# oleg-savchenko/jax_nbody_emulator_with_dj

Measured on AMD Instinct MI355X. Metric: voxels/sec (disp+vel) on 512^3 box, ndiv=4, higher is better.
Workload: dtype f32-equivalent: f16x3 split MFMA (3 f16 MFMAs per product, f32 accumulate)

## Files before the change

jax_nbody_emulator_with_dj_amd/csrc/nbe_kernels_head.h:

```cpp
constexpr int HNZ_ZRUN = 32;
constexpr int HNZ_MAXCH = 4;
constexpr int HNZ_R = 4;
constexpr int HNZ_TAPU = 4 * HNZ_R;
constexpr int HNZ_WG = 9 * HNZ_TAPU;
constexpr int HNZ_WC = 3 * HNZ_WG;
constexpr int HNZ_WS = 2 * HNZ_TAPU;
constexpr int HNZ_SBASE = HNZ_MAXCH * HNZ_WC;
constexpr int HNZ_XBASE = HNZ_SBASE + HNZ_MAXCH * HNZ_WS;
constexpr int HNZ_LDS_UNITS = HNZ_XBASE + 2 * HQ_XB;
constexpr int HNZ_SP = HP_ROWS * HP_COLS;
static_assert(8 * HNZ_SP <= HQ_XB, "the skip's patch fits a patch buffer");

__global__ __launch_bounds__(512, 1) void conv_h3nz_kernel(ConvKArgs a) {
    constexpr int R = HNZ_R, TAPU = HNZ_TAPU, WG = HNZ_WG, WC = HNZ_WC, XBASE = HNZ_XBASE, NT = 2, NW = 8;
    f32x4* lds = lds_h3;
    const half8* L8 = (const half8*)lds_h3;
    const int tid = threadIdx.x;
    const int lane = tid & 63;
    const int wave = __builtin_amdgcn_readfirstlane(tid >> 6);
    const int c = lane & 15, q = lane >> 4, kh = q & 1, ks = q >> 1;

    const int nrun = (a.Dv + a.zrun - 1) / a.zrun;
    const int tile = xcd_tile(blockIdx.x, a.ntiles);
    const int zr = tile % nrun, tyx = tile / nrun;
    const int ty = tyx / a.tnx, tx = tyx - ty * a.tnx;
    const int y0 = ty * HP_ROWS, x0 = tx * HP_COLS, z0 = zr * a.zrun;
    const int zn = min(a.zrun, a.Dv - z0);
    const int nchunk = a.nchunk, nskip = a.nskip;
    const long plane = (long)a.H * a.W * 16;
    const long to = (((long)z0 * a.H + y0) * a.W + x0) * 16;

    unsigned xoff[3];
    bool xval[3];
#pragma unroll
    for (int t = 0; t < 3; ++t) {
        const int k = (wave + NW * t) % 6;
        const int u = k * 64 + lane;
        xval[t] = u < HP_PL;
        const int uu = xval[t] ? u : HP_PL - 1;
        const int row = uu / HP_RS, col = uu - row * HP_RS;
        xoff[t] = (unsigned)(row * a.W + col) * 16u;
    }
    const unsigned soff = (unsigned)((2 * (wave & 3) + (lane >> 5) + 1) * a.W + (lane & 31) + 1) * 16u;
    auto fetch = [&](int p, int k, int buf) {
        const ConvGroupSrc e = a.gs[k];
        const char* xs = e.x + to + (long)p * plane;
        const char* dxs = e.dx + to + (long)p * plane;
        f32x4* xb = lds + XBASE + buf * HQ_XB;
        if (k < nchunk) {
#pragma unroll
            for (int t = 0; t < 3; ++t) {
                const int n = wave + NW * t, pl = n / 6, kk = n - 6 * pl;
                if (xval[t]) {
                    dma16s(xs + (long)pl * e.psb, xoff[t], xb + pl * HQ_PP + kk * 64);
                    dma16s(dxs + (long)pl * e.psb, xoff[t], xb + HQ_XT + pl * HQ_PP + kk * 64);
                }
            }
        } else {
#pragma unroll
            for (int t = 0; t < 2; ++t) {
                const int n = wave + NW * t, pl = n >> 2, kk = n & 3;
                dma16s(xs + (long)pl * e.psb, soff, xb + pl * HNZ_SP + kk * 64);
                dma16s(dxs + (long)pl * e.psb, soff, xb + 4 * HNZ_SP + pl * HNZ_SP + kk * 64);
            }
        }
    };

    {
        const int nmain = nchunk * WC;
        for (int n = wave; n * 64 < nmain; n += NW) {
            const int d = n * 64 + lane;
            if (d < nmain) dma16((const float*)((const char*)a.w + ((long)(d >> 2) * 16 + (d & 3)) * 16), lds + n * 64);
        }
        const int nsk = nskip * HNZ_WS;
        for (int n = wave; n * 64 < nsk; n += NW) {
            const int d = n * 64 + lane, sc = d >> 5, set = (d >> 4) & 1, r = d & 15;
            if (d < nsk)
                dma16((const float*)((const char*)a.ws + (set ? a.dws_delta : 0) + ((long)sc * 64 + (r >> 2) * 16 + (r & 3)) * 16),
                      lds + HNZ_SBASE + n * 64);
        }
    }

    f32x4 ym[NT], yc[NT], dm[NT], dc[NT];
    f32x4 ry[NT], rd[NT];
#pragma unroll
    for (int t = 0; t < NT; ++t)
#pragma unroll
        for (int e = 0; e < 4; ++e) { ym[t][e] = 0.f; yc[t][e] = 0.f; dm[t][e] = 0.f; dc[t][e] = 0.f; ry[t][e] = 0.f; rd[t][e] = 0.f; }
    auto mm = [&](f32x4& acc, const half8& A, const half8& B) { acc = __builtin_amdgcn_mfma_f32_16x16x32_f16(A, B, acc, 0, 0, 0); };

    const int rowp = wave;
    const int arow = min(c >> 2, 2) * WG + (c & 3);
    const int aP = (ks * 4 + 2 * kh) * R + arow;
    const int bB = (2 * kh) * HQ_PP + rowp * HP_RS + c;
    const int bP1 = bB + ks, bP32 = bB + 32 * ks;
    constexpr int SH4 = HP_RS + 1, SH5 = HP_RS + 2, SH7 = 2 * HP_RS + 1;
    const half8 zero = {0, 0, 0, 0, 0, 0, 0, 0};

    auto group = [&](int wb, int xb) {
        auto pair = [&](int wa, int xp) {
            const half8 wh = L8[wa + aP], wl = L8[wa + R + aP];
#pragma unroll
            for (int nt = 0; nt < NT; ++nt) {
                const half8 xh = L8[xp + 16 * nt], xl = L8[xp + HQ_PP + 16 * nt];
                const half8 dxh = L8[xp + HQ_XT + 16 * nt], dxl = L8[xp + HQ_XT + HQ_PP + 16 * nt];
                mm(yc[nt], wh, xl); mm(ym[nt], wh, xh); mm(dm[nt], wh, dxh);
                mm(dc[nt], wh, dxl); mm(yc[nt], wl, xh); mm(dc[nt], wl, dxh);
            }
            __builtin_amdgcn_sched_barrier(0);
        };
        pair(wb, xb + bP1);
        pair(wb + 2 * TAPU, xb + 2 + bP32);
        {
            const half8 a1w = L8[wb + 4 * TAPU + (2 * kh + ks) * R + arow];
            half8 a0 = L8[wb + 4 * TAPU + (2 * kh) * R + arow];
            a0 = ks ? a0 : zero;
            const int bS1 = xb + (2 * kh + 1 - ks) * HQ_PP + rowp * HP_RS + c + SH4;
#pragma unroll
            for (int nt = 0; nt < NT; ++nt) {
                const half8 b1x = L8[bS1 + 16 * nt], b1d = L8[bS1 + HQ_XT + 16 * nt];
                mm(yc[nt], a1w, b1x); mm(ym[nt], a0, b1x); mm(dc[nt], a1w, b1d); mm(dm[nt], a0, b1d);
            }
            __builtin_amdgcn_sched_barrier(0);
        }
        pair(wb + 5 * TAPU, xb + SH5 + bP32);
        pair(wb + 7 * TAPU, xb + SH7 + bP1);
    };
    auto skipgroup = [&](int wb, int xb) {
        const bool r03 = c < R;
        half8 a1w = L8[wb + (2 * kh + ks) * R + (c & 3)], a1d = L8[wb + TAPU + (2 * kh + ks) * R + (c & 3)];
        half8 a0 = L8[wb + (2 * kh) * R + (c & 3)], a0d = L8[wb + TAPU + (2 * kh) * R + (c & 3)];
        a1w = r03 ? a1w : zero; a1d = r03 ? a1d : zero;
        a0 = (r03 && ks) ? a0 : zero; a0d = (r03 && ks) ? a0d : zero;
        const int bS1 = xb + (2 * kh + 1 - ks) * HNZ_SP + rowp * HP_COLS + c;
#pragma unroll
        for (int nt = 0; nt < NT; ++nt) {
            const half8 b1x = L8[bS1 + 16 * nt], b1d = L8[bS1 + 4 * HNZ_SP + 16 * nt];
            mm(yc[nt], a1w, b1x); mm(ym[nt], a0, b1x);
            mm(dc[nt], a1w, b1d); mm(dm[nt], a0, b1d);
            mm(dc[nt], a1d, b1x); mm(dm[nt], a0d, b1x);
        }
    };

    const bool act = a.flags & F_ACT, gauge = a.gout != nullptr;
    float bv[8], be[8], gv[8];
#pragma unroll
    for (int j = 0; j < 8; ++j) { bv[j] = a.bias[j]; be[j] = a.beta[j]; gv[j] = gauge ? a.gout[j] : 0.f; }
    const int up16 = ((lane - 16) & 63) * 4;
    auto retire = [&](int pp) {
#pragma unroll
        for (int nt = 0; nt < NT; ++nt)
#pragma unroll
            for (int e = 0; e < 4; ++e) {
                const float ty = ym[nt][e] + yc[nt][e] * H3_INV, td = dm[nt][e] + dc[nt][e] * H3_INV;
                const float oy = ry[nt][e], od = rd[nt][e];
                const float sy = __int_as_float(__builtin_amdgcn_ds_bpermute(up16, __float_as_int(oy)));
                const float sd = __int_as_float(__builtin_amdgcn_ds_bpermute(up16, __float_as_int(od)));
                ry[nt][e] = (q ? sy : 0.f) + ty;
                rd[nt][e] = (q ? sd : 0.f) + td;
            }
        if (pp < 2 || q != 2) return;
        const int z = z0 + pp - 2;
#pragma unroll
        for (int nt = 0; nt < NT; ++nt) {
            const int yy = y0 + rowp, xx = x0 + 16 * nt + c;
            if (!(yy < a.Hv && xx < a.Wv)) continue;
            const long o = ((long)z * a.Ho + yy) * a.Wo + xx;
            half4 vh[2], vl[2], dh[2], dl[2];
#pragma unroll
            for (int h = 0; h < 2; ++h) {
                f32x4 v, dv;
#pragma unroll
                for (int e = 0; e < 4; ++e) {
                    const int j = 4 * h + e;
                    const float yp = h ? 0.f : ry[nt][e];
                    v[e] = yp + bv[j];
                    dv[e] = (h ? 0.f : rd[nt][e]) + be[j] * yp;
                    if (act) {
                        dv[e] = v[e] > 0.f ? dv[e] : 0.01f * dv[e];
                        v[e] = v[e] >= 0.f ? v[e] : 0.01f * v[e];
                    }
                    if (gauge) dv[e] += gv[j] * v[e];
                }
                split4(v, vh[h], vl[h]);
                split4(dv, dh[h], dl[h]);
            }
            const long ob = ((long)a.out_g0 * a.out_pstride + o) * 16;
            const long ol = ob + a.out_pstride * 16;
            struct alignas(16) H8 { half4 c03, c47; };
            *(H8*)((char*)a.y + ob) = H8{vh[0], vh[1]};
            *(H8*)((char*)a.y + ol) = H8{vl[0], vl[1]};
            *(H8*)((char*)a.dy + ob) = H8{dh[0], dh[1]};
            *(H8*)((char*)a.dy + ol) = H8{dl[0], dl[1]};
        }
    };

    fetch(0, 0, 0);
    asm volatile("s_waitcnt vmcnt(0)" ::: "memory");
    __syncthreads();
    int s = 0;
    for (int p = 0; p < zn + 2; ++p) {
        const int nk = nchunk + (p < zn ? nskip : 0);
        for (int k = 0; k < nk; ++k, ++s) {
            const bool last = k + 1 == nk;
            if (!last || p + 1 < zn + 2) fetch(last ? p + 1 : p, last ? 0 : k + 1, (s + 1) & 1);
            if (k == 0 && p > 0) {
                retire(p - 1);
#pragma unroll
                for (int t = 0; t < NT; ++t)
#pragma unroll
                    for (int e = 0; e < 4; ++e) { ym[t][e] = 0.f; yc[t][e] = 0.f; dm[t][e] = 0.f; dc[t][e] = 0.f; }
            }
            const int xb = XBASE + (s & 1) * HQ_XB;
            if (k < nchunk) group(k * WC, xb);
            else skipgroup(HNZ_SBASE + (k - nchunk) * HNZ_WS, xb);
            asm volatile("s_waitcnt vmcnt(0) lgkmcnt(0)" ::: "memory");
            __syncthreads();
        }
    }
    retire(zn + 1);
}

static int launch_h3nz(ConvKArgs ka, int ctiles, int cout, hipStream_t s) {
    constexpr size_t smem = (size_t)HNZ_LDS_UNITS * 16;
    static_assert(smem <= 160 * 1024, "LDS budget of one CU");
    if (ctiles != 1 || cout > HNZ_R || ka.cout_groups != 1 || (ka.flags & (F_RES | F_SKIP_NODX)) || !ka.beta || ka.Dv < 1) return 1;
    if (ka.nchunk > HNZ_MAXCH || ka.nskip > HNZ_MAXCH || ka.nchunk + ka.nskip > NBE_MAX_GROUPS) return 1;
    ensure_lds_limit((const void*)conv_h3nz_kernel, smem);
    ka.tny = (ka.Hv + HP_ROWS - 1) / HP_ROWS;
    ka.tnx = (ka.Wv + HP_COLS - 1) / HP_COLS;
    const int nrun = (ka.Dv + HNZ_ZRUN - 1) / HNZ_ZRUN;
    ka.zrun = (ka.Dv + nrun - 1) / nrun;
    ka.ntiles = ((ka.Dv + ka.zrun - 1) / ka.zrun) * ka.tny * ka.tnx;
    for (int chunk = 0; chunk < ka.nchunk; ++chunk) {
        const bool second = chunk >= ka.csplit;
        const long ps = second ? ka.in2_pstride : ka.in_pstride;
        const long off = (long)(second ? chunk - ka.csplit : chunk) * 4 * ps * 16;
        ka.gs[chunk] = {(const char*)(second ? ka.x2 : ka.x) + off, (const char*)(second ? ka.dx2 : ka.dx) + off,
                        (const char*)ka.w, ps * 16};
    }
    for (int sc = 0; sc < ka.nskip; ++sc) {
        const bool second = sc >= ka.s_csplit;
        const long ps = second ? ka.s2_pstride : ka.s_pstride;
        const long off = (long)(second ? sc - ka.s_csplit : sc) * 4 * ps * 16;
        ka.gs[ka.nchunk + sc] = {(const char*)(second ? ka.xs2 : ka.xs) + off, (const char*)(second ? ka.dxs2 : ka.dxs) + off,
                                 (const char*)ka.ws, ps * 16};
    }
    ka.dws_delta = ka.nskip ? (const char*)ka.dws - (const char*)ka.ws : 0;
    hipLaunchKernelGGL(conv_h3nz_kernel, dim3(ka.ntiles), dim3(512), smem, s, ka);
    return 0;
}
```

Baseline: 102.4 million.

## Triple-buffer patch fetches with partial vmcnt waits in head conv kernel

Moves the patch staging in the fused head conv kernel from double to triple buffering. Fetches now run two stages ahead, and each stage waits only until the newest fetch's loads may remain outstanding (vmcnt 6 or 4, hard-coded per fetch type) before the barrier. The aim is to keep global loads in flight across barriers instead of draining the memory queue every stage. The cost is one more patch buffer of LDS and a dependence on exact per-fetch load counts matching the immediates; retire() stores also count against vmcnt.

Measured after the change: 101.9 million. No clear change (-0.5%).

```diff
diff --git a/jax_nbody_emulator_with_dj_amd/csrc/nbe_kernels_head.h b/jax_nbody_emulator_with_dj_amd/csrc/nbe_kernels_head.h
--- a/jax_nbody_emulator_with_dj_amd/csrc/nbe_kernels_head.h
+++ b/jax_nbody_emulator_with_dj_amd/csrc/nbe_kernels_head.h
@@ -1,4 +1,5 @@
 constexpr int HNZ_ZRUN = 32;
+constexpr int HNZ_DMA_MAIN = 6, HNZ_DMA_SKIP = 4;
 constexpr int HNZ_MAXCH = 4;
 constexpr int HNZ_R = 4;
 constexpr int HNZ_TAPU = 4 * HNZ_R;
@@ -7,7 +8,7 @@
 constexpr int HNZ_WS = 2 * HNZ_TAPU;
 constexpr int HNZ_SBASE = HNZ_MAXCH * HNZ_WC;
 constexpr int HNZ_XBASE = HNZ_SBASE + HNZ_MAXCH * HNZ_WS;
-constexpr int HNZ_LDS_UNITS = HNZ_XBASE + 2 * HQ_XB;
+constexpr int HNZ_LDS_UNITS = HNZ_XBASE + 3 * HQ_XB;
 constexpr int HNZ_SP = HP_ROWS * HP_COLS;
 static_assert(8 * HNZ_SP <= HQ_XB, "the skip's patch fits a patch buffer");
 
@@ -195,15 +196,28 @@
         }
     };
 
-    fetch(0, 0, 0);
-    asm volatile("s_waitcnt vmcnt(0)" ::: "memory");
-    __syncthreads();
-    int s = 0;
+    int fp = 0, fk = 0, fb = 0;
+    auto fetch_next = [&]() -> int {
+        if (fp == zn + 2) return 0;
+        const int n = fk < nchunk ? HNZ_DMA_MAIN : HNZ_DMA_SKIP;
+        fetch(fp, fk, fb);
+        fb = fb == 2 ? 0 : fb + 1;
+        if (++fk == nchunk + (fp < zn ? nskip : 0)) { fk = 0; ++fp; }
+        return n;
+    };
+    auto stage_end = [&](int keep) {
+        if (keep == HNZ_DMA_MAIN) asm volatile("s_waitcnt vmcnt(6) lgkmcnt(0)\n\ts_barrier" ::: "memory");
+        else if (keep == HNZ_DMA_SKIP) asm volatile("s_waitcnt vmcnt(4) lgkmcnt(0)\n\ts_barrier" ::: "memory");
+        else asm volatile("s_waitcnt vmcnt(0) lgkmcnt(0)\n\ts_barrier" ::: "memory");
+    };
+    static_assert(HNZ_DMA_MAIN == 6 && HNZ_DMA_SKIP == 4, "the immediates of stage_end");
+
+    fetch_next();
+    stage_end(fetch_next());
+    int rb = 0;
     for (int p = 0; p < zn + 2; ++p) {
         const int nk = nchunk + (p < zn ? nskip : 0);
-        for (int k = 0; k < nk; ++k, ++s) {
-            const bool last = k + 1 == nk;
-            if (!last || p + 1 < zn + 2) fetch(last ? p + 1 : p, last ? 0 : k + 1, (s + 1) & 1);
+        for (int k = 0; k < nk; ++k) {
             if (k == 0 && p > 0) {
                 retire(p - 1);
 #pragma unroll
@@ -211,11 +225,12 @@
 #pragma unroll
                     for (int e = 0; e < 4; ++e) { ym[t][e] = 0.f; yc[t][e] = 0.f; dm[t][e] = 0.f; dc[t][e] = 0.f; }
             }
-            const int xb = XBASE + (s & 1) * HQ_XB;
+            const int keep = fetch_next();
+            const int xb = XBASE + rb * HQ_XB;
             if (k < nchunk) group(k * WC, xb);
             else skipgroup(HNZ_SBASE + (k - nchunk) * HNZ_WS, xb);
-            asm volatile("s_waitcnt vmcnt(0) lgkmcnt(0)" ::: "memory");
-            __syncthreads();
+            stage_end(keep);
+            rb = rb == 2 ? 0 : rb + 1;
         }
     }
     retire(zn + 1);
```
